# woolgathering/pyPeriod

Measured on AMD Instinct MI355X. Metric: window-projections/sec (all-p sweep, N=4096), higher is better.
Workload: dtype f64

## Files before the change

### pyperiod_amd/csrc/period_hip.hip

```cpp
#include <hip/hip_runtime.h>

#include <algorithm>
#include <cstdarg>
#include <cstdio>
#include <cstdlib>
#include <cstring>
#include <string>
#include <vector>

#include "../../include/periodhip.h"
#include "ph_kernels.h"
#include "ph_fit.h"
#include "ph_frames.h"

namespace {

thread_local std::string g_err;

int fail(int code, const char* fmt, ...) {
  char buf[512];
  va_list ap;
  va_start(ap, fmt);
  vsnprintf(buf, sizeof buf, fmt, ap);
  va_end(ap);
  g_err = buf;
  return code;
}

#define PH_HIP(call)                                                                         \
  do {                                                                                       \
    hipError_t e_ = (call);                                                                  \
    if (e_ != hipSuccess)                                                                    \
      return fail(e_ == hipErrorOutOfMemory ? PH_E_NOMEM : PH_E_HIP, "%s failed: %s", #call, \
                  hipGetErrorString(e_));                                                    \
  } while (0)

#define PH_TRY(expr)          \
  do {                        \
    int rc_ = (expr);         \
    if (rc_ != PH_OK) return rc_; \
  } while (0)

struct DevBuf {
  void* p = nullptr;
  size_t cap = 0;
};

struct TableSlot {
  DevBuf dev;
  std::vector<int32_t> host;
  bool valid = false;
};

enum { T_PLIST, T_ORTH_OFF, T_ORTH_Q, T_FAC_OFF, T_FAC_Q, T_AUX0, T_AUX1, T_AUX2, T_AUX3, T_FIT_PHI, T_FIT_OFF, T_FIT_DQ, T_COUNT };
enum { B_IN, B_OUT0, B_OUT1, B_OUT2, B_OUT3, B_OUT4, B_WS0, B_WS1, B_GEN0, B_GBUF, B_GWIN, B_COUNT };

}

struct ph_ctx {
  int device = 0;
  hipStream_t own_stream = nullptr;
  hipStream_t stream = nullptr;
  hipEvent_t ev0 = nullptr, ev1 = nullptr;
  int num_cu = 0;
  int lds_limit = 0;
  DevBuf buf[B_COUNT];
  TableSlot tab[T_COUNT];
  DevBuf geom;
  DevBuf geomf;
  DevBuf radq;
  DevBuf kapf;
  int geom_n = -1, geom_max_p = -1;
  bool step1_pair = true;
  bool s2l_pair = true;
  bool bc_pair = true;
  bool pair_chain = true;
  bool pair_cover = true;
  bool pair_duo = true;
  DevBuf twid;
  int twid_len = -1;
  DevBuf bs_tab;
  int bs_L = -1, bs_M0 = -1;
  DevBuf plan;
  int plan_lo = -1, plan_hi = -1, plan_n = 0, plan_m = -1, plan_duo_n = 0;
  int plan_max_m = 4;
  int sweep_block = ph::kBlockWide;
  int step1_block = 0;
  int qo_block = 1024;
  int s2l_block = 1024;
  bool qo_hbm_window = false;
  bool hbm_window = false;
  int mob_max_p = -1;
  std::vector<int32_t> mob_off, mob_d, mob_mu;
  bool prof_on = false;
  int prof_n = 0;
  std::vector<hipEvent_t> prof_ev;
  std::vector<const char*> prof_name;
};

namespace {

int ensure(ph_ctx* c, DevBuf& b, size_t bytes) {
  if (bytes <= b.cap && b.p) return PH_OK;
  if (b.p) {
    PH_HIP(hipStreamSynchronize(c->stream));
    PH_HIP(hipFree(b.p));
    b.p = nullptr;
    b.cap = 0;
  }
  const size_t want = std::max<size_t>(bytes, 256);
  PH_HIP(hipMalloc(&b.p, want));
  b.cap = want;
  return PH_OK;
}

int upload_table(ph_ctx* c, int slot, const int32_t* src, size_t n, const int** dev_out) {
  TableSlot& t = c->tab[slot];
  if (n == 0) {
    PH_TRY(ensure(c, t.dev, 16));
    *dev_out = static_cast<const int*>(t.dev.p);
    return PH_OK;
  }
  if (t.valid && t.host.size() == n && std::memcmp(t.host.data(), src, n * sizeof(int32_t)) == 0) {
    *dev_out = static_cast<const int*>(t.dev.p);
    return PH_OK;
  }
  t.valid = false;
  PH_HIP(hipStreamSynchronize(c->stream));
  PH_TRY(ensure(c, t.dev, n * sizeof(int32_t) + 256));
  t.host.assign(src, src + n);
  PH_HIP(hipMemcpyAsync(t.dev.p, t.host.data(), n * sizeof(int32_t), hipMemcpyHostToDevice, c->stream));
  PH_HIP(hipStreamSynchronize(c->stream));
  t.valid = true;
  *dev_out = static_cast<const int*>(t.dev.p);
  return PH_OK;
}

size_t elem_size(int dtype) { return dtype == PH_F64 ? 8 : 4; }

std::vector<ph::PassPlan> build_plan(int p_lo, int p_hi, int max_m, bool mixed = true, bool chains = false, int duo_n = 0) {
  std::vector<ph::PassPlan> host;
  std::vector<char> covered((size_t)p_hi + 1, 0);
  if (chains) {
    for (int L = std::min(p_hi, 64); L >= p_lo; --L) {
      if (covered[L]) continue;
      int n = 0;
      for (int q = L; q >= p_lo && q >= 1 && !covered[q]; q >>= 1) {
        covered[q] = 1;
        n += 1;
        if (q & 1) break;
      }
      host.push_back(ph::PassPlan{L, 8 + n});
    }
    std::reverse(host.begin(), host.end());
  }
  for (int p = p_lo; p <= p_hi; ++p) {
    if (p < 64 && !chains) {
      host.push_back(ph::PassPlan{p, 0});
      continue;
    }
    if (covered[p]) continue;
// ... 772 lines not shown
}


struct PairWs {
  double* gwin;
  const ph::PGeomF* geomf;
  const double* radq;
  const float* kapf;
};

int pair_workspace(ph_ctx* c, int64_t W, int N, PairWs* ws) {
  PH_TRY(ensure(c, c->buf[B_GWIN], (size_t)W * ph::win_stride((size_t)N) * sizeof(double)));
  *ws = PairWs{static_cast<double*>(c->buf[B_GWIN].p), static_cast<const ph::PGeomF*>(c->geomf.p),
               static_cast<const double*>(c->radq.p), static_cast<const float*>(c->kapf.p)};
  return PH_OK;
}

}


extern "C" {

int ph_version(void) { return PH_VERSION; }

#ifdef PH_CLOCKS
int ph_debug_stamps(long long* dst, int n_wg) {
  PH_HIP(hipDeviceSynchronize());
  PH_HIP(hipMemcpyFromSymbol(dst, HIP_SYMBOL(ph::g_ph_stamps), sizeof(long long) * 4 * (size_t)n_wg));
  return PH_OK;
}
#endif

const char* ph_last_error(void) { return g_err.c_str(); }

int ph_device_count(int* count) {
  if (!count) return fail(PH_E_ARG, "count is NULL");
  int n = 0;
  hipError_t e = hipGetDeviceCount(&n);
  if (e != hipSuccess) {
    *count = 0;
    return fail(PH_E_HIP, "hipGetDeviceCount: %s", hipGetErrorString(e));
  }
  *count = n;
  return PH_OK;
}

int ph_create(int device, ph_ctx** out) {
  if (!out) return fail(PH_E_ARG, "out is NULL");
  *out = nullptr;
  int n = 0;
  PH_HIP(hipGetDeviceCount(&n));
  if (device < 0 || device >= n) return fail(PH_E_ARG, "device %d not in [0, %d)", device, n);
  PH_HIP(hipSetDevice(device));
  ph_ctx* c = new (std::nothrow) ph_ctx();
  if (!c) return fail(PH_E_NOMEM, "out of host memory");
  c->device = device;
  hipDeviceProp_t prop;
  hipError_t e = hipGetDeviceProperties(&prop, device);
  if (e != hipSuccess) {
    delete c;
    return fail(PH_E_HIP, "hipGetDeviceProperties: %s", hipGetErrorString(e));
  }
  c->num_cu = prop.multiProcessorCount;
  size_t lds = prop.sharedMemPerBlock;
  lds = std::max(lds, prop.sharedMemPerBlockOptin);
  lds = std::max(lds, prop.maxSharedMemoryPerMultiProcessor);
  c->lds_limit = (int)std::min<size_t>(lds, 160 * 1024);
  if ((e = hipStreamCreateWithFlags(&c->own_stream, hipStreamNonBlocking)) != hipSuccess ||
      (e = hipEventCreate(&c->ev0)) != hipSuccess || (e = hipEventCreate(&c->ev1)) != hipSuccess) {
    delete c;
    return fail(PH_E_HIP, "stream/event creation: %s", hipGetErrorString(e));
  }
  c->stream = c->own_stream;
  if (const char* e = std::getenv("PH_PLAN_MAX_M")) {
    const int v = std::atoi(e);
    if (v == 1 || v == 2 || v == 4) c->plan_max_m = v;
  }
  if (const char* e = std::getenv("PH_STEP1_PAIR")) c->step1_pair = std::atoi(e) != 0;
  if (const char* e = std::getenv("PH_S2L_PAIR")) c->s2l_pair = std::atoi(e) != 0;
  if (const char* e = std::getenv("PH_BC_PAIR")) c->bc_pair = std::atoi(e) != 0;
  if (const char* e = std::getenv("PH_PAIR_CHAIN")) c->pair_chain = std::atoi(e) != 0;
  if (const char* e = std::getenv("PH_PAIR_COVER")) c->pair_cover = std::atoi(e) != 0;
  if (const char* e = std::getenv("PH_PAIR_DUO")) c->pair_duo = std::atoi(e) != 0;
  if (const char* e = std::getenv("PH_STEP1_BLOCK")) {
    const int v = std::atoi(e);
    if (v >= 64 && v <= 1024 && v % 64 == 0) c->step1_block = v;
  }
  if (const char* e = std::getenv("PH_S2L_BLOCK")) {
    const int v = std::atoi(e);
    if (v >= 512 && v <= 1024 && v % 64 == 0) c->s2l_block = v;
  }
  if (const char* e = std::getenv("PH_QO_BLOCK")) {
    const int v = std::atoi(e);
    if (v >= 64 && v <= 1024 && v % 64 == 0) c->qo_block = v;
  }
  if (std::getenv("PH_QO_HBM_WINDOW")) c->qo_hbm_window = true;
  if (const char* e = std::getenv("PH_HBM_WINDOW"))
    if (std::atoi(e) != 0) c->hbm_window = c->qo_hbm_window = true;
  if (const char* e = std::getenv("PH_SWEEP_BLOCK")) {
    const int v = std::atoi(e);
    if (v >= 64 && v <= 512 && v % 64 == 0) c->sweep_block = v;
  }
  *out = c;
  return PH_OK;
}

int ph_destroy(ph_ctx* c) {
  if (!c) return PH_OK;
  (void)hipSetDevice(c->device);
  (void)hipStreamSynchronize(c->stream);
  for (DevBuf& b : c->buf)
    if (b.p) (void)hipFree(b.p);
  for (TableSlot& t : c->tab)
    if (t.dev.p) (void)hipFree(t.dev.p);
  if (c->geom.p) (void)hipFree(c->geom.p);
  if (c->geomf.p) (void)hipFree(c->geomf.p);
  if (c->radq.p) (void)hipFree(c->radq.p);
  if (c->kapf.p) (void)hipFree(c->kapf.p);
  if (c->plan.p) (void)hipFree(c->plan.p);
  if (c->twid.p) (void)hipFree(c->twid.p);
  if (c->bs_tab.p) (void)hipFree(c->bs_tab.p);
  for (hipEvent_t e : c->prof_ev) (void)hipEventDestroy(e);
  if (c->ev0) (void)hipEventDestroy(c->ev0);
  if (c->ev1) (void)hipEventDestroy(c->ev1);
  if (c->own_stream) (void)hipStreamDestroy(c->own_stream);
  delete c;
  return PH_OK;
}

int ph_set_stream(ph_ctx* c, void* hip_stream) {
  if (!c) return fail(PH_E_ARG, "ctx is NULL");
  const hipError_t e = hipStreamSynchronize(c->stream);
  if (hip_stream == PH_STREAM_DEFAULT)
    c->stream = nullptr;
  else
    c->stream = hip_stream ? static_cast<hipStream_t>(hip_stream) : c->own_stream;
  if (e != hipSuccess) {
    (void)hipGetLastError();
    return fail(PH_E_HIP, "ph_set_stream: draining the previous stream failed (%s); the new stream is bound",
                hipGetErrorString(e));
  }
  return PH_OK;
}

int ph_sweep_plan_info(ph_ctx* c, int p_lo, int p_hi, int* n_pass, int* n_periods) {
  if (!c || !n_pass || !n_periods) return fail(PH_E_ARG, "NULL argument");
  PH_TRY(check_sweep_range(p_lo, p_hi));
  *n_pass = (int)build_plan(p_lo, p_hi, c->plan_max_m, true, c->pair_chain).size();
  *n_periods = p_hi - p_lo + 1;
  return PH_OK;
}

int ph_pair_radius_table(int N, int max_p, double* out) {
  if (!out) return fail(PH_E_ARG, "NULL argument");
  if (N < 1 || max_p < 1 || max_p > N) return fail(PH_E_ARG, "need 1 <= max_p <= N (got %d, %d)", max_p, N);
  const std::vector<double> host = pair_radius_table(N, max_p);
  std::copy(host.begin(), host.end(), out);
  return PH_OK;
}

int ph_m_best_info(ph_ctx* c, int dtype, int N, int num, int min_length, int max_length, unsigned flags,
                   int* windows_per_workgroup, int* lds_bytes_per_sample) {
  if (!c || !windows_per_workgroup || !lds_bytes_per_sample) return fail(PH_E_ARG, "NULL argument");
  MBestArgs a;
  PH_TRY(m_best_query(c, dtype, N, num, min_length, max_length, 0, flags, &a));
  *windows_per_workgroup = a.pair ? 2 : 1;
// ... 251 lines not shown
  const bool general = pl.k[0].second != PH_PLAN_NONE;
  const size_t lds = pl.k[0].lds;
  const int P = p_hi - p_lo + 1;
  const int sweep_block = pl.k[0].block;
  const int chunks = pick_chunks(c, W, P, 8 * (sweep_block / 64));
  void *gbuf, *gwin;
  PH_TRY(place(c, pl.k[0].second, B_GBUF, (size_t)W * chunks * N * sz, &gbuf));
  PH_TRY(place(c, pl.k[0].window, B_GWIN, (size_t)W * chunks * ph::win_stride(N + kPad) * sz, &gwin));
  const ph::PGeom* geom;
  PH_TRY(prepare_geom(c, N, p_hi, &geom));
  const ph::PassPlan* plan;
  int n_pass;
  PH_TRY(prepare_plan(c, p_lo, p_hi, &plan, &n_pass, 4, true, true));
  ph::Tables tb{};
  PH_TRY(prepare_orth(c, general ? flags : 0u, orth_off, orth_q, table_max_p, p_hi, &tb));
  Stage st(c, flags);
  const void* dx;
  void* dout;
  PH_TRY(st.in(x, (size_t)W * N * sz, &dx));
  PH_TRY(st.out(B_OUT0, out, (size_t)W * P * sizeof(double), &dout));
  const unsigned kflags = flags & (PH_FLAG_TRUNC | PH_FLAG_ORTH);
  const dim3 grid((unsigned)(W * chunks));
  PH_TRY(dispatch(dtype, !gwin, [&](auto t, auto lw) {
    using T = decltype(t);
    return launch(c, "k_sweep", ph::k_sweep<T, decltype(lw)::value>, grid, sweep_block, lds, (const T*)dx, N, p_lo, p_hi,
                  mode, chunks, kflags, tb, geom, plan, n_pass, (T*)gbuf, (T*)gwin, (double*)dout);
  }));
  return st.finish();
}

int ph_m_best(ph_ctx* c, const void* x, int dtype, int64_t W, int N, int num, int min_length, int max_length,
              int gamma, const int32_t* orth_off, const int32_t* orth_q, const int32_t* fac_off,
              const int32_t* fac_q, int table_max_p, unsigned flags, uint32_t* periods, double* powers,
              void* bases, int32_t* status, int32_t* n_sweeps) {
  PH_TRY(check_common(c, x, dtype, W, N));
  if (!periods || !powers || !bases || !status) return fail(PH_E_ARG, "output pointer is NULL");
  if (!fac_off || !fac_q) return fail(PH_E_ARG, "fac_off/fac_q tables are required");
  MBestArgs a;
  PH_TRY(resolve_m_best(c, dtype, N, num, min_length, max_length, gamma, fac_off, table_max_p, -1, flags, &a));
  max_length = a.max_length;
  const int max_fac = a.max_fac, p_scr = a.p_scr;
  const bool pair = a.pair;
  const KernelPlan &s1 = a.pl.k[0], &s2 = a.pl.k[1];
  PH_HIP(hipSetDevice(c->device));
  const size_t sz = elem_size(dtype);
  const int P = max_length - min_length + 1;
  void *gbuf1, *gbuf2, *gwin1, *gwin2;
  PH_TRY(place(c, s1.second, B_GBUF, (size_t)W * N * sz, &gbuf1));
  PH_TRY(place(c, s2.second, B_GBUF, (size_t)W * N * sz, &gbuf2));
  PH_TRY(place(c, s1.window, B_GWIN, (size_t)W * ph::win_stride(N + kPad) * sz, &gwin1));
  PH_TRY(place(c, s2.window, B_GWIN, (size_t)W * ph::win_stride(N + kPad) * sz, &gwin2));
  ph::Tables tb{};
  PH_TRY(prepare_orth(c, flags, orth_off, orth_q, table_max_p, max_length, &tb));
  PH_TRY(prepare_fac(c, fac_off, fac_q, table_max_p, max_length, &tb));
  const ph::PGeom* geom;
  PH_TRY(prepare_geom(c, N, max_length, &geom));
  const ph::PassPlan* plan;
  int n_pass;
  PH_TRY(prepare_plan(c, p_scr, max_length, &plan, &n_pass, 4, false, pair, pair ? N : 0));
  Stage st(c, flags);
  const void* dx;
  void *dper, *dpow, *dbases, *dstat;
  PH_TRY(st.in(x, (size_t)W * N * sz, &dx));
  PH_TRY(st.out(B_OUT0, periods, (size_t)W * num * sizeof(uint32_t), &dper));
  PH_TRY(st.out(B_OUT1, powers, (size_t)W * num * sizeof(double), &dpow));
  PH_TRY(st.out(B_OUT2, bases, (size_t)W * num * N * sz, &dbases));
  PH_TRY(st.out(B_OUT3, status, (size_t)W * sizeof(int32_t), &dstat));
  void* dsweeps;
  PH_TRY(st.out(B_OUT4, n_sweeps, (size_t)W * sizeof(int32_t), &dsweeps));
  PH_TRY(ensure(c, c->buf[B_WS0], (size_t)W * sizeof(double)));
  double* dnorm = static_cast<double*>(c->buf[B_WS0].p);
  const int row_stride = (max_length + 127) & ~127;
  PH_TRY(ensure(c, c->buf[B_WS1], (size_t)W * num * row_stride * sz));
  void* drows = c->buf[B_WS1].p;
  const unsigned kflags = flags & (PH_FLAG_TRUNC | PH_FLAG_ORTH);
  const int max_iters = 12 * (P + num) + 64;
  const dim3 grid((unsigned)W);
  if (pair) {
    PairWs ws;
    PH_TRY(pair_workspace(c, W, N, &ws));
    PH_TRY(launch(c, "k_mbest_step1", ph::k_mbest_step1_pair, dim3((unsigned)((W + 1) / 2)), s1.block, s1.lds,
                  (const double*)dx, (int)W, N, num, min_length, max_length, p_scr, gamma, tb.fac_off, tb.fac_q, geom, ws.geomf,
                  ws.radq, plan, n_pass, ws.gwin, max_iters, (uint32_t*)dper, (double*)dpow, (double*)drows, row_stride, dnorm,
                  (int*)dstat, (int*)dsweeps));
  } else {
    PH_TRY(dispatch(dtype, !gwin1, [&](auto t, auto lw) {
      using T = decltype(t);
      return launch(c, "k_mbest_step1", ph::k_mbest_step1<T, decltype(lw)::value>, grid, s1.block, s1.lds, (const T*)dx, N,
                    num, min_length, max_length, gamma, kflags, tb, geom, plan, n_pass, (T*)gbuf1, (T*)gwin1, max_iters,
                    (uint32_t*)dper, (double*)dpow, (T*)drows, row_stride, dnorm, (int*)dstat, (int*)dsweeps,
                    s1.small_means);
    }));
  }
  PH_TRY(dispatch(dtype, !gwin2, [&](auto t, auto lw) {
    using T = decltype(t);
    return launch(c, "k_mbest_step2", ph::k_mbest_step2<T, decltype(lw)::value>, grid, s2.block, s2.lds, N, num, gamma,
                  max_length, kflags, tb, geom, max_fac, (T*)gbuf2, (T*)gwin2, (uint32_t*)dper, (double*)dpow, (T*)dbases,
                  dnorm, (const int*)dstat, (T*)drows, row_stride);
  }));
  return st.finish();
}

int ph_small_to_large(ph_ctx* c, const void* x, int dtype, int64_t W, int N, double thresh, int n_periods,
                      const int32_t* orth_off, const int32_t* orth_q, int table_max_p, unsigned flags, int cap,
                      int32_t* counts, int32_t* periods, double* powers, void* bases, int32_t* status) {
  PH_TRY(check_common(c, x, dtype, W, N));
  if (!counts || !periods || !powers || !status) return fail(PH_E_ARG, "output pointer is NULL");
  if (cap < 1) return fail(PH_E_ARG, "cap=%d must be >= 1", cap);
  Plan pl;
  PH_TRY(resolve_small_to_large(c, dtype, N, &n_periods, flags, &pl));
  PH_HIP(hipSetDevice(c->device));
  const size_t sz = elem_size(dtype);
  const KernelPlan& k = pl.k[0];
  void *gbuf, *gwin;
  PH_TRY(place(c, k.second, B_GBUF, (size_t)W * N * sz, &gbuf));
  PH_TRY(place(c, k.window, B_GWIN, (size_t)W * ph::win_stride(N + kPad) * sz, &gwin));
  const ph::PGeom* geom;
  PH_TRY(prepare_geom(c, N, std::max(n_periods, 2), &geom));
  ph::Tables tb{};
  PH_TRY(prepare_orth(c, flags, orth_off, orth_q, table_max_p, std::max(n_periods, 1), &tb));
  Stage st(c, flags);
  const void* dx;
  void *dcnt, *dper, *dpow, *dbases, *dstat;
  PH_TRY(st.in(x, (size_t)W * N * sz, &dx));
  PH_TRY(st.out(B_OUT0, counts, (size_t)W * sizeof(int32_t), &dcnt));
  PH_TRY(st.out(B_OUT1, periods, (size_t)W * cap * sizeof(int32_t), &dper));
  PH_TRY(st.out(B_OUT2, powers, (size_t)W * cap * sizeof(double), &dpow));
  PH_TRY(st.out(B_OUT3, bases, (size_t)W * cap * N * sz, &dbases));
  PH_TRY(st.out(B_OUT4, status, (size_t)W * sizeof(int32_t), &dstat));
  PH_HIP(hipMemsetAsync(dper, 0, (size_t)W * cap * sizeof(int32_t), c->stream));
  PH_HIP(hipMemsetAsync(dpow, 0, (size_t)W * cap * sizeof(double), c->stream));
  PH_TRY(ensure(c, c->buf[B_GEN0], 256));
  int* dmax = static_cast<int*>(c->buf[B_GEN0].p);
  PH_HIP(hipMemsetAsync(dmax, 0, 2 * sizeof(int), c->stream));
  const unsigned kflags = flags & (PH_FLAG_TRUNC | PH_FLAG_ORTH);
  const dim3 grid((unsigned)W);
  if (k.variant == PH_PLAN_PAIR) {
    PairWs ws;
    PH_TRY(pair_workspace(c, W, N, &ws));
    const int64_t npairs = (W + 1) / 2;
    const int per_cu = (int)std::max<size_t>(1, std::min<size_t>((size_t)c->lds_limit / k.lds, 2048 / (size_t)k.block));
    const unsigned grid_pairs = (unsigned)std::min<int64_t>(npairs, (int64_t)c->num_cu * per_cu);
    PH_TRY(launch(c, "k_small_to_large", ph::k_small_to_large_pair, dim3(grid_pairs), k.block, k.lds, (const double*)dx,
                  (int)W, N, thresh, n_periods, ws.geomf, ws.kapf, ws.gwin, cap, (int*)dcnt, (int*)dper, (double*)dpow,
                  (double*)dbases, (int*)dstat, dmax, dmax + 1));
  } else {
    PH_TRY(dispatch(dtype, !gwin, [&](auto t, auto lw) {
      using T = decltype(t);
      return launch(c, "k_small_to_large", ph::k_small_to_large<T, decltype(lw)::value>, grid, k.block, k.lds, (const T*)dx,
                    N, thresh, n_periods, kflags, tb, geom, (T*)gbuf, (T*)gwin, cap, (int*)dcnt, (int*)dper, (double*)dpow,
                    (T*)dbases, (int*)dstat, dmax);
    }));
  }
  PH_TRY(st.finish());
  if (!(flags & PH_FLAG_DEVICE) || !(flags & PH_FLAG_NOSYNC)) {
    int worst = 0;
    PH_HIP(hipMemcpyAsync(&worst, dmax, sizeof(int), hipMemcpyDeviceToHost, c->stream));
    PH_HIP(hipStreamSynchronize(c->stream));
    if (worst > cap) return fail(PH_E_CAP, "a window accepted %d periods, cap is %d", worst, cap);
  }
  return PH_OK;
}

int ph_best_correlation(ph_ctx* c, const void* x, int dtype, int64_t W, int N, int num, int max_length,
                        double ratio, const int32_t* orth_off, const int32_t* orth_q, int table_max_p,
                        unsigned flags, uint32_t* periods, double* norms, void* bases, int32_t* status) {
  PH_TRY(check_common(c, x, dtype, W, N));
// ... 1025 lines not shown
```

### pyperiod_amd/csrc/ph_mbest.h

```cpp
#pragma once

#include "ph_device.h"
#include "ph_pair.h"

namespace ph {

__device__ __forceinline__ bool skip_test(const uint32_t* skip, int i) { return (skip[i >> 5] >> (i & 31)) & 1u; }
__device__ __forceinline__ void skip_set(uint32_t* skip, int i) { skip[i >> 5] |= 1u << (i & 31); }

template <typename Norm>
__device__ __forceinline__ bool mbest_prefers(double ss, int p, double best_ss, int bestp, int gamma, Norm&& norm) {
  bool take = bestp == 0;
  if (!take) {
    const double lhs = gamma ? ss * (double)bestp : ss;
    const double rhs = gamma ? best_ss * (double)p : best_ss;
    if (lhs > rhs * (1.0 + 1e-14)) {
      take = true;
    } else if (lhs >= rhs * (1.0 - 1e-14)) {
      const double vn = norm(ss, gamma ? p : 0);
      const double vb = norm(best_ss, gamma ? bestp : 0);
      take = vn > vb || (vn == vb && p < bestp);
    }
  }
  return take;
// ... 150 lines not shown
      split_row_means(work, msm, prt, N, bestp, tid, min((int)blockDim.x, kPairSplitW));
      if (tid < bestp) {
        const T m = msm[tid];
        if (action == 1)
          brow[tid] = m;
        else if (action == 2)
          brow[tid] += m;
      }
      int idx = tid % bestp;
      const int step = blockDim.x % bestp;
      for (int n = tid; n < N; n += blockDim.x) {
        work[n] -= msm[idx];
        idx += step;
        idx = idx >= bestp ? idx - bestp : idx;
      }
    } else if (!general) {
      const Fold f(N, bestp);
      for (int j = tid; j < bestp; j += blockDim.x) {
        const T m = residue_mean(work, f, j, false);
        const int cnt = f.count(j);
        if (action == 1)
          brow[j] = m;
        else if (action == 2)
          brow[j] += m;
        for (int r = 0; r < cnt; ++r) work[r * bestp + j] -= m;
      }
    } else {
      project_lds(work, buf, N, bestp, flags, tb);
      for (int n = tid; n < N; n += blockDim.x) {
        const T m = buf[n];
        if (n < bestp) {
          if (action == 1)
            brow[n] = m;
          else if (action == 2)
            brow[n] += m;
        }
        work[n] -= m;
      }
    }
    __syncthreads();
  }
  __syncthreads();
  for (int k = tid; k < num; k += blockDim.x) {
    periods_out[w * num + k] = periods[k];
    norms_out[w * num + k] = norms[k];
  }
  if (tid == 0) {
    dnorm_out[w] = data_norm;
    status_out[w] = status;
    if (sweeps_out) sweeps_out[w] = status == 2 ? iters - 1 : iters;
  }
}

constexpr int kPairCoop = 6;

enum {
  MP_LISTED = 0,
  MP_FILLED = 2,
  MP_REPEATS = 4,
  MP_STATUS = 6,
  MP_SWEEPS = 8,
  MP_RUNNING = 10,
  MP_EXACT_ALL = 12,
  MP_QUEUE = 14,
  MP_WORDS = 16
};
enum { MP_UNIT = 0, MP_SCALE = 2, MP_DOUBLES = 4 };

__device__ __forceinline__ double pair_exact_part(const double* __restrict__ xs, int p, const PGeom& g, int first, int stride) {
  double part = 0.0;
  for (int j = first; j < p; j += stride) {
    const bool full = j < g.nfull;
    const double s = column_sum(xs, j, p, full ? g.rows : g.rows - 1);
    part = fma(s * s, full ? g.w_full : g.w_short, part);
  }
  return part;
}

__global__ __launch_bounds__(1024) __attribute__((amdgpu_waves_per_eu(PH_STEP1_WAVES, 8))) void k_mbest_step1_pair(
    const double* __restrict__ x, int W, int N, int num, int p_lo, int p_hi, int p_scr, int gamma,
    const int* __restrict__ fac_off, const int* __restrict__ fac_q, const PGeom* __restrict__ geom, const PGeomF* __restrict__ geomf, const double* __restrict__ radq, const PassPlan* __restrict__ plan, int n_pass,
    double* __restrict__ gres, int max_iters, uint32_t* __restrict__ periods_out, double* __restrict__ norms_out,
    double* __restrict__ rows_out, int row_stride, double* __restrict__ dnorm_out, int* __restrict__ status_out,
    int* __restrict__ sweeps_out) {
  extern __shared__ __attribute__((aligned(16))) unsigned char smem[];
  Carve cv(smem);
  f2* pw = cv.take<f2>(N + kPad);
  double* stg = cv.take<double>(N + kPad);
  double* red = cv.take<double>(kRedDoubles);
  double* wbest = cv.take<double>(kMaxWaves);
  int* wbestp = cv.take<int>(kMaxWaves);
  double* norms = cv.take<double>(2 * num);
  uint32_t* periods = cv.take<uint32_t>(2 * num);
  const int P = p_hi - p_lo + 1;
  const int SK = (P + 31) / 32;
  uint32_t* skip = cv.take<uint32_t>(2 * SK);
  int* list = cv.take<int>(2 * kPairListCap);
  int* ctl = cv.take<int>(MP_WORDS);
  double* dst2 = cv.take<double>(MP_DOUBLES);
  double* msm = cv.take<double>(kPairSmallP);
  double* prt = cv.take<double>(kPairSplitW);

  const int tid = threadIdx.x;
  const int wv = __builtin_amdgcn_readfirstlane(tid >> 6);
  const int nw = blockDim.x >> 6;
  const size_t gstride = win_stride((size_t)N);
  float* pwf = reinterpret_cast<float*>(pw);
  const double sqrtN = uniform_f64(sqrt((double)N));

  for (int k = tid; k < 2 * num; k += blockDim.x) {
    norms[k] = 0.0;
    periods[k] = 0u;
  }
  for (int k = tid; k < 2 * SK; k += blockDim.x) skip[k] = 0u;
  if (tid < MP_WORDS) ctl[tid] = tid == MP_QUEUE ? nw : 0;
  zero_pad(stg, N);
  for (int i = tid; i < kPad; i += blockDim.x) pw[N + i] = f2_zero();
  for (int w = 0; w < 2; ++w) {
    const int64_t gw = 2 * (int64_t)blockIdx.x + w;
    const bool exists = gw < W;
    __syncthreads();
    if (exists) {
      load_window(x + gw * (int64_t)N, stg, N);
    } else {
      for (int n = tid; n < N; n += blockDim.x) stg[n] = 0.0;
    }
    __syncthreads();
    const double rsq = block_sumsq(stg, N, red);
    const double sc = uniform_f64(pair_pick_scale(rsq, N));
    for (int n = tid; n < N; n += blockDim.x) pwf[2 * n + w] = (float)(stg[n] * sc);
    if (tid == 0) {
      dst2[MP_UNIT + w] = rsq * sc * sc * (1.0 + 1e-9);
      dst2[MP_SCALE + w] = sc;
      ctl[MP_RUNNING + w] = exists ? 1 : 0;
      ctl[MP_EXACT_ALL + w] = pair_usable(rsq) ? 0 : 1;
      if (exists) dnorm_out[gw] = periodic_norm_from_sq_n(rsq, sqrtN, 0);
    }
  }
  StageClock<kPairTimers, 5, 2> clk;
  WgStamp<kClocks> stamp;
  for (;;) {
    __syncthreads();
    const bool act0 = __builtin_amdgcn_readfirstlane(ctl[MP_RUNNING]) != 0, act1 = __builtin_amdgcn_readfirstlane(ctl[MP_RUNNING + 1]) != 0;
    if (!act0 && !act1) break;
    prio_by_progress(__builtin_amdgcn_readfirstlane(max(ctl[MP_SWEEPS], ctl[MP_SWEEPS + 1])));
    if (wv == 0 && pair_lane() == 0) ctl[MP_LISTED] = ctl[MP_LISTED + 1] = 0;
    f2* vals = reinterpret_cast<f2*>(stg);
    pair_sweep_plan<false, true>(
        pw, N, geomf, plan, wv, n_pass, nw, [&](float z, int q) { pair_store1(vals, z, q, p_lo); },
        [&](float z, int q_a, int q_b) { pair_store2(vals, z, q_a, q_b, p_lo); },
        PH_PAIR_QUEUE ? &ctl[MP_QUEUE] : nullptr);
    __syncthreads();
    clk.mark(0);
    prio_short_phase();
    {
    const int tid = (wv << 6) + pair_lane();
    const int lane = tid & (kWave - 1);
    if (tid == 0) ctl[MP_QUEUE] = nw;
    {
      const bool scr0 = act0 && !__builtin_amdgcn_readfirstlane(ctl[MP_EXACT_ALL]), scr1 = act1 && !__builtin_amdgcn_readfirstlane(ctl[MP_EXACT_ALL + 1]);
      if (scr0 || scr1) {
        const double unit0 = uniform_f64(dst2[MP_UNIT]), unit1 = uniform_f64(dst2[MP_UNIT + 1]);
        const int i0 = p_scr - p_lo;
        const bool cover = i0 > 0;
        const int SD = (i0 + 31) >> 5;
        uint32_t* seen = reinterpret_cast<uint32_t*>(stg);
        for (int k = tid; k < 2 * SD; k += blockDim.x) seen[k] = 0u;
        const double slack = cover ? pair_cover_slack(N) : 0.0;
        struct Entry {
          f2 v;
          double rad, rq;
          bool skip0, skip1;
        };
        auto entry = [&](int idx) {
          Entry e;
          const int q = p_lo + idx;
          const uint32_t bit = 1u << (idx & 31);
          e.v = vals[idx];
          e.rad = radq[q];
          e.rq = gamma ? 1.0 / (double)q : 1.0;
          e.skip0 = (skip[idx >> 5] & bit) != 0;
          e.skip1 = (skip[SK + (idx >> 5)] & bit) != 0;
          return e;
        };
        const int idx_own = i0 + tid;
        Entry own = {f2_zero(), 0.0, 1.0, true, true};
        if (idx_own < P) own = entry(idx_own);
        double lo0 = -1.0 / 0.0, lo1 = -1.0 / 0.0;
        for (int idx = idx_own; idx < P; idx += blockDim.x) {
          const Entry e = idx == idx_own ? own : entry(idx);
          double a = (double)e.v.x - e.rad * unit0, b = (double)e.v.y - e.rad * unit1;
          if (gamma) {
            a *= e.rq;
            b *= e.rq;
          }
          if (!e.skip0 && a > lo0) lo0 = a;
          if (!e.skip1 && b > lo1) lo1 = b;
        }
        lo0 = wave_max(lo0);
        lo1 = wave_max(lo1);
        if (lane == 0) {
          red[wv] = lo0;
          red[kMaxWaves + wv] = lo1;
        }
        __syncthreads();
        lo0 = uniform_f64(red_combine<true>(red, nw));
        lo1 = uniform_f64(red_combine<true>(red + kMaxWaves, nw));
        const bool none0 = cover && scr0 && !(lo0 > -1.0 / 0.0), none1 = cover && scr1 && !(lo1 > -1.0 / 0.0);
        if (tid == 0 && none0) ctl[MP_LISTED] = kPairListCap + 1;
        if (tid == 0 && none1) ctl[MP_LISTED + 1] = kPairListCap + 1;
        const double thr0 = lo0 - fabs(lo0) * 1e-9, thr1 = lo1 - fabs(lo1) * 1e-9;
        for (int idx = idx_own; idx < P; idx += blockDim.x) {
          const Entry e = idx == idx_own ? own : entry(idx);
          const int q = p_lo + idx;
          const double rad = e.rad + slack;
          double a = (double)e.v.x + rad * unit0, b = (double)e.v.y + rad * unit1;
          if (gamma) {
            a *= e.rq;
            b *= e.rq;
          }
          const bool hit0 = scr0 && !none0 && a >= thr0, hit1 = scr1 && !none1 && b >= thr1;
          if (hit0 && !e.skip0) {
            const int k = atomicAdd(&ctl[MP_LISTED], 1);
            if (k < kPairListCap) list[k] = q;
          }
          if (hit1 && !e.skip1) {
            const int k = atomicAdd(&ctl[MP_LISTED + 1], 1);
            if (k < kPairListCap) list[kPairListCap + k] = q;
          }
          if (cover && (hit0 || hit1)) {
            const int f1 = fac_off[q + 1];
            for (int f = fac_off[q] - (p_lo == 1 ? 1 : 0); f < f1; ++f) {
              const int d = f < fac_off[q] ? 1 : fac_q[f];
              if (d < p_lo || d >= p_scr) continue;
              const int di = d - p_lo;
              const uint32_t dbit = 1u << (di & 31);
              for (int w = 0; w < 2; ++w) {
                if (!(w ? hit1 : hit0) || (skip[w * SK + (di >> 5)] & dbit)) continue;
                if (atomicOr(&seen[w * SD + (di >> 5)], dbit) & dbit) continue;
                const int k = atomicAdd(&ctl[MP_LISTED + w], 1);
                if (k < kPairListCap) list[w * kPairListCap + k] = d;
              }
            }
          }
        }
      }
    }
    __syncthreads();
    clk.mark(1);
    for (int w = 0; w < 2; ++w) {
      if (!(w ? act1 : act0)) continue;
      const int64_t gw = 2 * (int64_t)blockIdx.x + w;
      int filled = __builtin_amdgcn_readfirstlane(ctl[MP_FILLED + w]), repeats = __builtin_amdgcn_readfirstlane(ctl[MP_REPEATS + w]), status = 0,
          iters = __builtin_amdgcn_readfirstlane(ctl[MP_SWEEPS + w]);
      const int nlisted = __builtin_amdgcn_readfirstlane(ctl[MP_LISTED + w]);
      const bool exact_all = __builtin_amdgcn_readfirstlane(ctl[MP_EXACT_ALL + w]) != 0 || nlisted > kPairListCap;
      int ncand = exact_all ? P : nlisted;
      double* nrm = norms + w * num;
      uint32_t* per = periods + w * num;
      uint32_t* sk = skip + w * SK;
      const int* lst = list + w * kPairListCap;
      __syncthreads();
      if (iters + 1 > max_iters) {
        status = 2;
      } else {
        const double* src = iters == 0 ? x + gw * (int64_t)N : gres + gw * gstride;
        iters += 1;
        load_window(src, stg, N);
        __syncthreads();
        clk.mark(2);
        if (kPairTimers) {
          clk.count(0, ncand);
          clk.count(1, exact_all ? 1 : 0);
        }
        if (p_scr > p_lo && !exact_all && ncand > 1) {
          for (int k = wv; k < ncand; k += nw) {
            const int p = lst[k];
            const PGeom g = geom[p];
            const double part = p < 64 ? wave_partial_small(stg, N, p, g, lane) : pair_exact_part(stg, p, g, lane, kWave);
            const double ss = wave_sum(part);
            if (lane == 0) msm[k] = ss;
          }
          __syncthreads();
          if (wv == 0) {
            const int k0 = lane, k1 = kWave + lane;
            const double v0 = k0 < ncand ? msm[k0] : -1.0, v1 = k1 < ncand ? msm[k1] : -1.0;
            const int q0 = lst[k0], q1 = k1 < kPairListCap ? lst[k1] : 0;
            const double top = wave_max(fmax(v0, v1));
            const bool keep0 = k0 < ncand && v0 >= top - fabs(top) * 1e-9, keep1 = k1 < ncand && v1 >= top - fabs(top) * 1e-9;
            const unsigned long long m0 = __ballot(keep0), m1 = __ballot(keep1);
            const unsigned long long below = (1ull << lane) - 1ull;
            const int n0 = __popcll(m0);
            int* out = list + w * kPairListCap;
            if (keep0) out[__popcll(m0 & below)] = q0;
            if (keep1) out[n0 + __popcll(m1 & below)] = q1;
            if (lane == 0) ctl[MP_LISTED + w] = n0 + __popcll(m1);
          }
          __syncthreads();
          ncand = __builtin_amdgcn_readfirstlane(ctl[MP_LISTED + w]);
        }
        double best_ss = 0.0;
        int bestp = 0;
        const auto norm = [&](double s, int div) { return periodic_norm_from_sq_n(s, sqrtN, div); };
        auto consider = [&](double ss, int p) {
          if (!(ss > 0.0)) return;
          if (mbest_prefers(ss, p, best_ss, bestp, gamma, norm)) {
            best_ss = ss;
            bestp = p;
          }
        };
        double best = 0.0;
        if (ncand <= kPairCoop) {
          for (int k = 0; k < ncand; ++k) {
            const int p = exact_all ? p_lo + k : lst[k];
            if (skip_test(sk, p - p_lo)) continue;
            const PGeom g = geom[p];
            double part = 0.0;
            if (p < 64) {
              if (wv == 0) part = wave_partial_small(stg, N, p, g, lane);
            } else {
              part = pair_exact_part(stg, p, g, tid, blockDim.x);
            }
            consider(block_sum(part, red), p);
          }
          best = bestp != 0 ? periodic_norm_from_sq_n(best_ss, sqrtN, gamma ? bestp : 0) : 0.0;
          if (!(best > 0.0)) bestp = 0;
        } else {
          for (int k = wv; k < ncand; k += nw) {
            const int p = exact_all ? p_lo + k : lst[k];
            if (skip_test(sk, p - p_lo)) continue;
            const PGeom g = geom[p];
            const double part = p < 64 ? wave_partial_small(stg, N, p, g, lane) : pair_exact_part(stg, p, g, lane, kWave);
            consider(wave_sum(part), p);
          }
          best = bestp != 0 ? periodic_norm_from_sq_n(best_ss, sqrtN, gamma ? bestp : 0) : 0.0;
          if (!(best > 0.0)) bestp = 0;
          if (lane == 0) {
            wbest[wv] = best;
            wbestp[wv] = bestp;
          }
          __syncthreads();
          red_argmax(wbest, wbestp, nw, best, bestp);
          __syncthreads();
        }
        clk.mark(3);
        if (bestp == 0) {
          status = 1;
        } else {
          int row = -1;
          for (int k0 = 0; k0 < num; k0 += kWave) {
            const unsigned long long hit = __ballot(k0 + lane < num && per[k0 + lane] == (uint32_t)bestp);
            if (hit) row = k0 + 63 - __clzll(hit);
          }
          const int action = mbest_book(row, bestp, best, p_lo, tid, filled, repeats, nrm, per, sk);
          double* brow = rows_out + (gw * (int64_t)num + (row < 0 ? 0 : row)) * row_stride;
          const bool more = filled < num;
          const double sc = uniform_f64(dst2[MP_SCALE + w]);
          double* dst = gres + gw * gstride;
          double acc = 0.0;
          const PGeom gb = geom[__builtin_amdgcn_readfirstlane(bestp)];
          const Fold f(bestp, gb.rows, gb.nfull);
          if (bestp <= kPairSmallP) {
            split_row_means(stg, msm, prt, N, bestp, tid, kPairSplitW);
            if (tid < bestp) {
              const double m = msm[tid];
              if (action == 1)
                brow[tid] = m;
              else if (action == 2)
                brow[tid] += m;
            }
            if (more) {
              int idx = tid % bestp;
              const int step = blockDim.x % bestp;
              for (int n = tid; n < N; n += blockDim.x) {
                const double v = stg[n] - msm[idx];
                dst[n] = v;
                pwf[2 * n + w] = (float)(v * sc);
                acc = fma(v, v, acc);
                idx += step;
                idx = idx >= bestp ? idx - bestp : idx;
              }
            }
          } else {
            for (int j = tid; j < bestp; j += blockDim.x) {
              const double m = residue_mean(stg, f, j, false);
              const int cnt = f.count(j);
              if (action == 1)
                brow[j] = m;
              else if (action == 2)
                brow[j] += m;
              if (more) {
                for (int r = 0; r < cnt; ++r) {
                  const int n = r * bestp + j;
                  const double v = stg[n] - m;
                  dst[n] = v;
                  pwf[2 * n + w] = (float)(v * sc);
                  acc = fma(v, v, acc);
                }
              }
            }
          }
          if (more) {
            const double rsq = block_sum(acc, red);
            const double unit = rsq * sc * sc;
            const bool ok = pair_usable(rsq);
            if (pair_image_stale(rsq, sc, N)) {
              const double sc2 = uniform_f64(pair_pick_scale(rsq, N));
              __syncthreads();
              pair_rescale(pwf, w, N, (float)(sc2 / sc), tid);
              if (tid == 0) {
                dst2[MP_UNIT + w] = rsq * sc2 * sc2 * (1.0 + 1e-9);
                dst2[MP_SCALE + w] = sc2;
              }
            } else if (tid == 0) {
              dst2[MP_UNIT + w] = unit * (1.0 + 1e-9);
            }
            if (tid == 0) ctl[MP_EXACT_ALL + w] = ok ? 0 : 1;
          }
        }
      }
      __syncthreads();
      if (tid == 0) {
        ctl[MP_FILLED + w] = filled;
        ctl[MP_REPEATS + w] = repeats;
        ctl[MP_STATUS + w] = status;
        ctl[MP_SWEEPS + w] = iters;
        ctl[MP_RUNNING + w] = (status == 0 && filled < num) ? 1 : 0;
      }
      clk.mark(4);
    }
    }
  }
  if (kClocks && (blockIdx.x % 16) == 7 && tid == 0) {
    stamp.finish();
    printf("PAIRWG %d start %lld end %lld cycles %lld MHz %.0f hwid %x xcc %x\n", (int)blockIdx.x, stamp.wk0, stamp.wk1, stamp.ck1 - stamp.ck0,
           100.0 * (double)(stamp.ck1 - stamp.ck0) / (double)(stamp.wk1 - stamp.wk0), stamp.hwid, stamp.xcc);
  }
  if (kPairTimers && blockIdx.x < PH_PAIR_TIMERS_WGS && tid == 0)
    printf("pair timers (100 MHz ticks) screen %lld scan %lld load %lld exact %lld update %lld  candidates %d exact_all %d sweeps %d %d\n",
           clk.ticks(0), clk.ticks(1), clk.ticks(2), clk.ticks(3), clk.ticks(4), clk.counted(0), clk.counted(1), ctl[MP_SWEEPS], ctl[MP_SWEEPS + 1]);
  __syncthreads();
  for (int w = 0; w < 2; ++w) {
    const int64_t gw = 2 * (int64_t)blockIdx.x + w;
    if (gw >= W) continue;
    for (int k = tid; k < num; k += blockDim.x) {
      periods_out[gw * num + k] = periods[w * num + k];
      norms_out[gw * num + k] = norms[w * num + k];
    }
    if (tid == 0) {
      status_out[gw] = ctl[MP_STATUS + w];
      if (sweeps_out) sweeps_out[gw] = ctl[MP_SWEEPS + w];
    }
  }
}

__device__ __forceinline__ PGeom make_geom(int N, int p) {
  const int rows = (N + p - 1) / p;
  PGeom g;
  g.rows = rows;
  g.nfull = p - (rows * p - N);
  g.w_full = 1.0 / (double)rows;
  g.w_short = rows > 1 ? 1.0 / (double)(rows - 1) : 0.0;
  return g;
}

constexpr int kStep2Pre = 3;
typedef __attribute__((address_space(3))) void* lds_void_ptr;
typedef const __attribute__((address_space(1))) void* global_void_ptr;

template <typename T>
__device__ __forceinline__ void expand_row(const T* __restrict__ src, int p, T* __restrict__ dst, int N) {
  const int step = blockDim.x % p;
  int idx = threadIdx.x % p;
  for (int n = threadIdx.x; n < N; n += blockDim.x) {
    dst[n] = src[idx];
    idx += step;
    if (idx >= p) idx -= p;
  }
}

template <typename T, bool LW>
__global__ __launch_bounds__(kBlockWide) __attribute__((amdgpu_waves_per_eu(PH_STEP1_WAVES, 8))) void k_mbest_step2(int N, int num, int gamma, int stale_p, unsigned flags,
                                                        Tables tb, const PGeom* __restrict__ geom, int max_fac,
                                                        T* __restrict__ gbuf, T* gwin,
                                                        uint32_t* __restrict__ periods_io,
                                                        double* __restrict__ norms_io, T* __restrict__ bases_out,
                                                        const double* __restrict__ dnorm,
                                                        const int* __restrict__ status, T* __restrict__ rows_io,
                                                        int row_stride) {
  extern __shared__ __attribute__((aligned(16))) unsigned char smem[];
  Carve cv(smem);
  T* rowbuf = window_buf<T, LW>(cv, gwin, N + kPad);
  T* buf = gbuf ? gbuf + (int64_t)blockIdx.x * N : cv.take<T>(N);
  double* red = cv.take<double>(kRedDoubles);
  double* norms = cv.take<double>(num);
  uint32_t* periods = cv.take<uint32_t>(num);
  double* fvals = cv.take<double>(max_fac > 0 ? max_fac : 1);
  int* ffac = cv.take<int>(max_fac > 0 ? max_fac : 1);
  PGeom* fgeom = cv.take<PGeom>(kMaxWaves);
  int* fa = cv.take<int>(num);
  int* fb = cv.take<int>(num);
  int* slot = cv.take<int>(num);
  int* ffac_next = cv.take<int>(max_fac > 64 ? max_fac : 64);

  const int64_t w = blockIdx.x;
  const int tid = threadIdx.x;
  const int lane = tid & (kWave - 1);
  const int wv = __builtin_amdgcn_readfirstlane(tid >> 6);
  const int nw = blockDim.x >> 6;
  const bool general = flags & (kTrunc | kOrth);
  const bool periodic_rows = sizeof(T) == 8 && !general;
  T* rows = rows_io + w * (int64_t)num * row_stride;
  for (int k = tid; k < num; k += blockDim.x) {
    norms[k] = norms_io[w * num + k];
    const uint32_t per = periods_io[w * num + k];
    periods[k] = per;
    fa[k] = tb.fac_off[per];
    fb[k] = tb.fac_off[per + 1];
    slot[k] = k;
  }
  zero_pad(rowbuf, N);
  __syncthreads();

  StageClock<kStep2Timers, 6, 2> clk;
  const int gdiv = gamma ? stale_p : 0;
  int i = (status[w] == 0) ? 0 : num;
  auto next_row = [&](int r) {
    while (r < num && fa[r] == fb[r]) ++r;
    return r;
  };
  const T* stage = nullptr;
  int stage_row = -1;
  T* out = bases_out + w * (int64_t)num * N;
  int done = 0;
// ... 184 lines not shown
```

### pyperiod_amd/csrc/ph_pair.h

```cpp
#pragma once

#include "ph_device.h"

namespace ph {

typedef float f2 __attribute__((ext_vector_type(2)));
typedef const volatile __attribute__((address_space(3))) f2* pair_ptr;

struct PGeomF {
  int rows;
  int nfull;
  float w_full;
  float w_short;
};

__device__ __forceinline__ f2 f2_make(float a, float b) {
  f2 r;
  r.x = a;
  r.y = b;
  return r;
}
__device__ __forceinline__ f2 f2_zero() { return f2_make(0.0f, 0.0f); }
__device__ __forceinline__ f2 f2_fma(f2 a, f2 b, f2 c) { return __builtin_elementwise_fma(a, b, c); }
__device__ __forceinline__ f2 f2_max(f2 a, f2 b) { return __builtin_elementwise_max(a, b); }
// ... 568 lines not shown
template <bool MX, typename F, typename F2>
__device__ __forceinline__ void pair_chain_small(const f2* __restrict__ xs, int N, int L, int nlev,
                                                 const PGeomF* __restrict__ geom, F&& consume, F2&& consume2) {
  const int lane = pair_lane();
  PGeomF g = geom[L];
  const int full = g.nfull == L ? g.rows : g.rows - 1;
  const bool on = lane < L;
  const f2* ptr = xs + (on ? lane : 0);
  f2 s0 = f2_zero(), s1 = f2_zero();
  int r = 0;
  for (; r + 4 <= full; r += 4) {
    const f2 a = ptr[0], b = ptr[L], c = ptr[2 * L], d = ptr[3 * L];
    s0 += a;
    s1 += b;
    s0 += c;
    s1 += d;
    ptr += 4 * L;
  }
  for (; r < full; ++r) {
    s0 += ptr[0];
    ptr += L;
  }
  const bool tail = on && (full * L + lane < N);
  const f2 tv = xs[tail ? full * L + lane : 0];
  f2 tot = s0 + s1 + (tail ? tv : f2_zero());
  tot = on ? tot : f2_zero();
  int q = L;
  for (int lev = 0; lev < nlev; lev += 2) {
    const f2 va = pair_chain_term<MX>(tot, lane, q, g);
    if (lev + 1 < nlev) {
      const int q2 = q >> 1;
      const PGeomF g2 = geom[q2];
      tot += pair_shift_down(tot, lane, q2);
      const f2 vb = pair_chain_term<MX>(tot, lane, q2, g2);
      consume2(pair_reduce2<MX>(va, vb), q, q2);
      if (lev + 2 < nlev) {
        q = q2 >> 1;
        g = geom[q];
        tot += pair_shift_down(tot, lane, q);
      }
    } else {
      consume(pair_reduce1<MX>(va), q);
    }
  }
}

template <bool MX = false, bool DUO = false, typename F, typename F2>
__device__ __forceinline__ void pair_sweep_plan(const f2* __restrict__ xs, int N, const PGeomF* __restrict__ geom,
                                                const PassPlan* __restrict__ plan, int i_first, int i_end, int stride,
                                                F&& consume, F2&& consume2, int* __restrict__ queue = nullptr) {
  auto red = [](f2 v) { return pair_reduce1<MX>(v); };
  for (int i = i_first; i < i_end;) {
    int ticket = 0;
    if (queue && pair_lane() == 0) ticket = lds_ticket(queue);
    const int p = plan[i].p, m = plan[i].m;
    if (m >= 8) {
      pair_chain_small<MX>(xs, N, p, m - 8, geom, consume, consume2);
    } else if (m == 0) {
      consume(red(pair_partial_small<MX>(xs, N, p, geom[p])), p);
    } else if (m == 1) {
      consume(red(pair_pass_single<MX>(xs, p, geom[p])), p);
    } else if (DUO && m == 3) {
      f2 va, vb;
      pair_pass_duo(xs, N, p, geom[p], va, vb);
      consume2(pair_reduce2<MX>(va, vb), p, p + 64);
    } else if (m == 2) {
      f2 part[3];
      pair_pass_multi<2, MX>(xs, p, geom, part);
      consume2(pair_reduce2<MX>(part[0], part[1]), p, 2 * p);
    } else {
      f2 part[3];
      pair_pass_multi<4, MX>(xs, p, geom, part);
      consume2(pair_reduce2<MX>(part[0], part[1]), p, 2 * p);
      consume(red(part[2]), 4 * p);
    }
    i = queue ? lds_ticket_value(ticket) : i + stride;
  }
}

__host__ __device__ __forceinline__ double pair_radius(int rows, int q) {
  return 1.5 * (2.0 * (double)rows + (double)(q >> 6) + 32.0) * 5.9604644775390625e-08;
}

__device__ __forceinline__ double pair_cover_slack(int N) {
  return fmax(9.094947017729282e-13, (2.0 * (double)N + 32.0) * 2.220446049250313e-16);
}

#ifndef PH_PAIR_QUEUE
#define PH_PAIR_QUEUE 1
#endif
constexpr int kPairListCap = 96;
constexpr int kPairSmallP = 256;
constexpr int kPairSplitW = 512;

__device__ __forceinline__ bool pair_usable(double rsq) { return rsq > 0.0 && rsq < 1.79e308; }

__device__ __forceinline__ double pair_pick_scale(double rsq, int N) {
  if (!pair_usable(rsq)) return 1.0;
  int e;
  (void)frexp(rsq / (double)N, &e);
  return ldexp(1.0, -(e >> 1));
}

constexpr double kPairStaleMeanSq = 9.0e-13;
__device__ __forceinline__ bool pair_image_stale(double rsq, double sc, int N) {
  return pair_usable(rsq) && rsq * sc * sc < kPairStaleMeanSq * (double)N;
}

__device__ __forceinline__ void pair_rescale(float* __restrict__ pwf, int w, int N, float up, int tid = threadIdx.x) {
  for (int n = tid; n < N; n += blockDim.x) pwf[2 * n + w] *= up;
}

__device__ __forceinline__ int pair_rows_upper(float fn, int q) {
  return (int)(fn * __builtin_amdgcn_rcpf((float)q) * 1.000001f) + 1;
}

}
```

Before: 9.635 billion.

## Fold window by single large candidate period and screen divisors from folded sums

When exactly one screened candidate is at or above the screening threshold and every other candidate divides it, the pair step1 kernel computes column sums for that period directly from global memory. It then evaluates the divisor candidates from those folded sums against a thin tolerance band instead of loading the full window and running exact passes. If any divisor comes within the band, it falls back to the original path. This is meant to skip the full window load and the per-candidate exact projections in the common case, at the cost of strided global reads, an extra block reduction, and new bookkeeping packed into the status field.

New measurement: 9.900 billion (median of 6 runs). +2.8%, better.

```diff
diff --git a/pyperiod_amd/csrc/period_hip.hip b/pyperiod_amd/csrc/period_hip.hip
--- a/pyperiod_amd/csrc/period_hip.hip
+++ b/pyperiod_amd/csrc/period_hip.hip
@@ -77,6 +77,8 @@
   bool pair_chain = true;
   bool pair_cover = true;
   bool pair_duo = true;
+  bool pair_fold_once = true;
+  bool pair_fold_report = false;
   DevBuf twid;
   int twid_len = -1;
   DevBuf bs_tab;
@@ -1015,6 +1017,8 @@
   if (const char* e = std::getenv("PH_PAIR_CHAIN")) c->pair_chain = std::atoi(e) != 0;
   if (const char* e = std::getenv("PH_PAIR_COVER")) c->pair_cover = std::atoi(e) != 0;
   if (const char* e = std::getenv("PH_PAIR_DUO")) c->pair_duo = std::atoi(e) != 0;
+  if (const char* e = std::getenv("PH_PAIR_FOLD_ONCE")) c->pair_fold_once = std::atoi(e) != 0;
+  if (const char* e = std::getenv("PH_PAIR_FOLD_REPORT")) c->pair_fold_report = std::atoi(e) != 0;
   if (const char* e = std::getenv("PH_STEP1_BLOCK")) {
     const int v = std::atoi(e);
     if (v >= 64 && v <= 1024 && v % 64 == 0) c->step1_block = v;
@@ -1432,7 +1436,7 @@
     PH_TRY(launch(c, "k_mbest_step1", ph::k_mbest_step1_pair, dim3((unsigned)((W + 1) / 2)), s1.block, s1.lds,
                   (const double*)dx, (int)W, N, num, min_length, max_length, p_scr, gamma, tb.fac_off, tb.fac_q, geom, ws.geomf,
                   ws.radq, plan, n_pass, ws.gwin, max_iters, (uint32_t*)dper, (double*)dpow, (double*)drows, row_stride, dnorm,
-                  (int*)dstat, (int*)dsweeps));
+                  (int*)dstat, (int*)dsweeps, c->pair_fold_once ? ph::pair_thin_band(N) : -1.0, c->pair_fold_report ? 1 : 0));
   } else {
     PH_TRY(dispatch(dtype, !gwin1, [&](auto t, auto lw) {
       using T = decltype(t);
diff --git a/pyperiod_amd/csrc/ph_mbest.h b/pyperiod_amd/csrc/ph_mbest.h
--- a/pyperiod_amd/csrc/ph_mbest.h
+++ b/pyperiod_amd/csrc/ph_mbest.h
@@ -256,7 +256,8 @@
     const int* __restrict__ fac_off, const int* __restrict__ fac_q, const PGeom* __restrict__ geom, const PGeomF* __restrict__ geomf, const double* __restrict__ radq, const PassPlan* __restrict__ plan, int n_pass,
     double* __restrict__ gres, int max_iters, uint32_t* __restrict__ periods_out, double* __restrict__ norms_out,
     double* __restrict__ rows_out, int row_stride, double* __restrict__ dnorm_out, int* __restrict__ status_out,
-    int* __restrict__ sweeps_out) {
+    int* __restrict__ sweeps_out, double thin_band, int fold_report) {
+  const bool fold_once = __double2hiint(thin_band) >= 0;
   extern __shared__ __attribute__((aligned(16))) unsigned char smem[];
   Carve cv(smem);
   f2* pw = cv.take<f2>(N + kPad);
@@ -311,7 +312,7 @@
       if (exists) dnorm_out[gw] = periodic_norm_from_sq_n(rsq, sqrtN, 0);
     }
   }
-  StageClock<kPairTimers, 5, 2> clk;
+  StageClock<kPairTimers, 6, 3> clk;
   WgStamp<kClocks> stamp;
   for (;;) {
     __syncthreads();
@@ -435,18 +436,60 @@
       uint32_t* sk = skip + w * SK;
       const int* lst = list + w * kPairListCap;
       __syncthreads();
+      bool folded = false;
       if (iters + 1 > max_iters) {
         status = 2;
       } else {
         const double* src = iters == 0 ? x + gw * (int64_t)N : gres + gw * gstride;
         iters += 1;
+        int fold_m = 0;
+        double fold_ss = 0.0;
+        if (fold_once && !exact_all) {
+          const int k0 = lane, k1 = kWave + lane;
+          const int q0 = k0 < ncand ? lst[k0] : 0, q1 = k1 < ncand ? lst[k1] : 0;
+          const unsigned long long t0 = __ballot(q0 >= p_scr), t1 = __ballot(q1 >= p_scr);
+          if (__popcll(t0) + __popcll(t1) == 1) {
+            const int m = t0 ? __builtin_amdgcn_readlane(q0, __builtin_amdgcn_readfirstlane(__ffsll((long long)t0) - 1))
+                             : __builtin_amdgcn_readlane(q1, __builtin_amdgcn_readfirstlane(__ffsll((long long)t1) - 1));
+            const float fm = (float)m;
+            const int c0 = (int)(fm * __builtin_amdgcn_rcpf((float)max(q0, 1)) + 0.5f), c1 = (int)(fm * __builtin_amdgcn_rcpf((float)max(q1, 1)) + 0.5f);
+            const bool odd = (k0 < ncand && c0 * q0 != m) || (k1 < ncand && c1 * q1 != m);
+            if (m > kPairSmallP && __ballot(odd) == 0ull) fold_m = m;
+          }
+        }
+        if (fold_m != 0) {
+          const PGeom gm = geom[fold_m];
+          double part = 0.0;
+          if (tid == 0) wbestp[0] = 0;
+          for (int j = tid; j < fold_m; j += blockDim.x) {
+            const bool full = j < gm.nfull;
+            const double s = pair_column_sum_global(src, j, fold_m, full ? gm.rows : gm.rows - 1);
+            part = fma(s * s, full ? gm.w_full : gm.w_short, part);
+            stg[j] = s;
+          }
+          fold_ss = block_sum(part, red);
+          clk.mark(2);
+          if (ncand > 1) {
+            const int se = __builtin_amdgcn_frexp_exp(dst2[MP_SCALE + w]) - 1;
+            const double band = thin_band * ldexp(dst2[MP_UNIT + w], -2 * se);
+            double tie = 1e-9;
+            asm volatile("" : "+s"(tie));
+            const double thr = fold_ss - fabs(fold_ss) * tie - band;
+            for (int k = wv; k < ncand; k += nw) {
+              const int d = __builtin_amdgcn_readfirstlane(lst[k]);
+              if (d == fold_m) continue;
+              const double t = wave_sum(pair_thin_part(stg, fold_m, d, geom[d], lane));
+              if (lane == 0 && !(t < thr)) wbestp[0] = 1;
+            }
+            __syncthreads();
+            if (__builtin_amdgcn_readfirstlane(wbestp[0]) != 0) fold_m = 0;
+          }
+          clk.mark(3);
+        }
+        if (fold_m == 0) {
         load_window(src, stg, N);
         __syncthreads();
         clk.mark(2);
-        if (kPairTimers) {
-          clk.count(0, ncand);
-          clk.count(1, exact_all ? 1 : 0);
-        }
         if (p_scr > p_lo && !exact_all && ncand > 1) {
           for (int k = wv; k < ncand; k += nw) {
             const int p = lst[k];
@@ -473,6 +516,14 @@
           __syncthreads();
           ncand = __builtin_amdgcn_readfirstlane(ctl[MP_LISTED + w]);
         }
+        clk.mark(3);
+        }
+        folded = fold_m != 0;
+        if (kPairTimers) {
+          clk.count(0, exact_all ? P : nlisted);
+          clk.count(1, exact_all ? 1 : 0);
+          clk.count(2, fold_m != 0 ? 1 : 0);
+        }
         double best_ss = 0.0;
         int bestp = 0;
         const auto norm = [&](double s, int div) { return periodic_norm_from_sq_n(s, sqrtN, div); };
@@ -484,7 +535,11 @@
           }
         };
         double best = 0.0;
-        if (ncand <= kPairCoop) {
+        if (fold_m != 0) {
+          consider(fold_ss, fold_m);
+          best = bestp != 0 ? periodic_norm_from_sq_n(best_ss, sqrtN, gamma ? bestp : 0) : 0.0;
+          if (!(best > 0.0)) bestp = 0;
+        } else if (ncand <= kPairCoop) {
           for (int k = 0; k < ncand; ++k) {
             const int p = exact_all ? p_lo + k : lst[k];
             if (skip_test(sk, p - p_lo)) continue;
@@ -517,7 +572,7 @@
           red_argmax(wbest, wbestp, nw, best, bestp);
           __syncthreads();
         }
-        clk.mark(3);
+        clk.mark(4);
         if (bestp == 0) {
           status = 1;
         } else {
@@ -534,7 +589,34 @@
           double acc = 0.0;
           const PGeom gb = geom[__builtin_amdgcn_readfirstlane(bestp)];
           const Fold f(bestp, gb.rows, gb.nfull);
-          if (bestp <= kPairSmallP) {
+          if (fold_m != 0) {
+            for (int j = tid; j < bestp; j += blockDim.x) {
+              const int cnt = f.count(j);
+              const double m = stg[j] / (double)cnt;
+              if (action == 1)
+                brow[j] = m;
+              else if (action == 2)
+                brow[j] += m;
+              if (more) {
+                for (int r0 = 0; r0 < cnt; r0 += 4) {
+                  const unsigned at = (unsigned)(r0 * bestp + j);
+                  double v[4];
+#pragma unroll
+                  for (int u = 0; u < 4; ++u) v[u] = src[r0 + u < cnt ? at + (unsigned)(u * bestp) : at];
+#pragma unroll
+                  for (int u = 0; u < 4; ++u) {
+                    if (r0 + u < cnt) {
+                      const unsigned n = at + (unsigned)(u * bestp);
+                      const double t = v[u] - m;
+                      dst[n] = t;
+                      pwf[2 * n + w] = (float)(t * sc);
+                      acc = fma(t, t, acc);
+                    }
+                  }
+                }
+              }
+            }
+          } else if (bestp <= kPairSmallP) {
             split_row_means(stg, msm, prt, N, bestp, tid, kPairSplitW);
             if (tid < bestp) {
               const double m = msm[tid];
@@ -597,11 +679,11 @@
       if (tid == 0) {
         ctl[MP_FILLED + w] = filled;
         ctl[MP_REPEATS + w] = repeats;
-        ctl[MP_STATUS + w] = status;
+        ctl[MP_STATUS + w] = status | (((ctl[MP_STATUS + w] >> 8) + (folded ? 1 : 0)) << 8);
         ctl[MP_SWEEPS + w] = iters;
         ctl[MP_RUNNING + w] = (status == 0 && filled < num) ? 1 : 0;
       }
-      clk.mark(4);
+      clk.mark(5);
     }
     }
   }
@@ -611,8 +693,9 @@
            100.0 * (double)(stamp.ck1 - stamp.ck0) / (double)(stamp.wk1 - stamp.wk0), stamp.hwid, stamp.xcc);
   }
   if (kPairTimers && blockIdx.x < PH_PAIR_TIMERS_WGS && tid == 0)
-    printf("pair timers (100 MHz ticks) screen %lld scan %lld load %lld exact %lld update %lld  candidates %d exact_all %d sweeps %d %d\n",
-           clk.ticks(0), clk.ticks(1), clk.ticks(2), clk.ticks(3), clk.ticks(4), clk.counted(0), clk.counted(1), ctl[MP_SWEEPS], ctl[MP_SWEEPS + 1]);
+    printf("pair timers (100 MHz ticks) screen %lld scan %lld load %lld thin %lld exact %lld update %lld  candidates %d exact_all %d folded %d sweeps %d %d\n",
+           clk.ticks(0), clk.ticks(1), clk.ticks(2), clk.ticks(3), clk.ticks(4), clk.ticks(5), clk.counted(0), clk.counted(1), clk.counted(2), ctl[MP_SWEEPS],
+           ctl[MP_SWEEPS + 1]);
   __syncthreads();
   for (int w = 0; w < 2; ++w) {
     const int64_t gw = 2 * (int64_t)blockIdx.x + w;
@@ -622,8 +705,8 @@
       norms_out[gw * num + k] = norms[w * num + k];
     }
     if (tid == 0) {
-      status_out[gw] = ctl[MP_STATUS + w];
-      if (sweeps_out) sweeps_out[gw] = ctl[MP_SWEEPS + w];
+      status_out[gw] = ctl[MP_STATUS + w] & 255;
+      if (sweeps_out) sweeps_out[gw] = ctl[MP_SWEEPS + w] | (fold_report ? (ctl[MP_STATUS + w] >> 8) << 16 : 0);
     }
   }
 }
diff --git a/pyperiod_amd/csrc/ph_pair.h b/pyperiod_amd/csrc/ph_pair.h
--- a/pyperiod_amd/csrc/ph_pair.h
+++ b/pyperiod_amd/csrc/ph_pair.h
@@ -674,8 +674,61 @@
   return 1.5 * (2.0 * (double)rows + (double)(q >> 6) + 32.0) * 5.9604644775390625e-08;
 }
 
-__device__ __forceinline__ double pair_cover_slack(int N) {
+__host__ __device__ __forceinline__ double pair_cover_slack(int N) {
   return fmax(9.094947017729282e-13, (2.0 * (double)N + 32.0) * 2.220446049250313e-16);
+}
+
+__host__ __device__ __forceinline__ double pair_thin_band(int N) { return 5.0 * pair_cover_slack(N); }
+
+__device__ __forceinline__ double pair_column_sum_global(const double* __restrict__ src, int j, int m, int n) {
+  unsigned at = (unsigned)j;
+  double s = src[at];
+  at += (unsigned)m;
+  for (int r = 1; r < n; r += 4) {
+    const bool k1 = r + 1 < n, k2 = r + 2 < n, k3 = r + 3 < n;
+    const double a = src[at], b = src[k1 ? at + (unsigned)m : at], c = src[k2 ? at + 2u * (unsigned)m : at],
+                 d = src[k3 ? at + 3u * (unsigned)m : at];
+    s += a;
+    s = k1 ? s + b : s;
+    s = k2 ? s + c : s;
+    s = k3 ? s + d : s;
+    at += 4u * (unsigned)m;
+  }
+  return s;
+}
+
+__device__ __forceinline__ double pair_thin_part(const double* __restrict__ S, int m, int d, const PGeom& g, int lane) {
+  double part = 0.0;
+  if (d >= kWave) {
+    const int n = m / d;
+    for (int j0 = lane; j0 < d; j0 += 4 * kWave) {
+      double s[4];
+      const double* at = S + j0;
+#pragma unroll
+      for (int u = 0; u < 4; ++u) s[u] = at[j0 + u * kWave < d ? u * kWave : 0];
+      for (int r = 1; r < n; ++r) {
+        at += d;
+#pragma unroll
+        for (int u = 0; u < 4; ++u) s[u] += at[j0 + u * kWave < d ? u * kWave : 0];
+      }
+#pragma unroll
+      for (int u = 0; u < 4; ++u) {
+        const int j = j0 + u * kWave;
+        if (j < d) part = fma(s[u] * s[u], j < g.nfull ? g.w_full : g.w_short, part);
+      }
+    }
+  } else {
+    const int G = kWave / d, L = G * d;
+    const int q = m / L, rem = m - q * L;
+    double tot = lane < L ? column_sum(S, lane, L, q + (lane < rem ? 1 : 0)) : 0.0;
+    const double own = tot;
+    for (int k = 1; k < G; ++k) {
+      const double o = __shfl(own, (lane + k * d) & (kWave - 1), kWave);
+      tot += o;
+    }
+    part = lane < d ? tot * tot * (lane < g.nfull ? g.w_full : g.w_short) : 0.0;
+  }
+  return part;
 }
 
 #ifndef PH_PAIR_QUEUE
```
